# aagbotemi/zk-cryptography

Measured on AMD Instinct MI355X. Metric: field-evals/s (sumcheck 2^24) + MSM points/s (KZG 2^20) per BASELINE.json; value = the sumcheck prover's field-evals/s, the MSM half is under "msm", higher is better.
Workload: dtype u32; 1 GPU; 24-var multilinear sumcheck prover (poly_sum + prove), BLS12-381 Fr; field=BLS12-381 Fr (255-bit Montgomery, 8 x u32 limbs); G1 over Fq (381-bit), evals_per_gpu=16777216, exchanges_per_prove=0

## Files before the change

zk-cryptography_amd/csrc/ctx.hpp:

```cpp
#pragma once
#include <hip/hip_runtime.h>
#include <stdint.h>

#include <algorithm>
#include <deque>
#include <functional>
#include <memory>
#include <mutex>
#include <new>
#include <set>
#include <vector>

#include "../../include/zkhip.h"
#include "hip_own.hpp"
#include "host_util.hpp"

#define ZK_MAX_ROUNDS 48
#define ZK_MAX_PARTIALS 4096

enum : size_t {
    ZK_SMALL_R = 0,
    ZK_SMALL_RES = 16,
    ZK_SMALL_STATE = 64,
    ZK_SMALL_PTS = 256,
    ZK_SMALL_CHALLENGES = ZK_SMALL_PTS + 4 * ZK_MAX_ROUNDS,
    ZK_SMALL_ROUNDPOLYS = ZK_SMALL_CHALLENGES + 4 * ZK_MAX_ROUNDS,
    ZK_SMALL_PARTIALS = ZK_SMALL_ROUNDPOLYS + 64 * ZK_MAX_ROUNDS,
    ZK_SMALL_END = ZK_SMALL_PARTIALS + 4 * 8 * ZK_MAX_PARTIALS
};
#define ZK_SMALL_BYTES (ZK_SMALL_END * 8)

enum : size_t {
    ZK_PIN_R = 0,
    ZK_PIN_RES = 16,
    ZK_PIN_PTS = 64,
    ZK_PIN_PROOF = ZK_PIN_PTS + 4 * ZK_MAX_ROUNDS,
    ZK_PIN_END = ZK_PIN_PROOF + 4 + 8 * ZK_MAX_ROUNDS + 4 * ZK_MAX_ROUNDS + 64 * ZK_MAX_ROUNDS
};
#define ZK_PINNED_BYTES (ZK_PIN_END * 8)

#define ZK_HIP(ctx, call)                                   \
    do {                                                    \
        hipError_t _e = (call);                             \
        if (_e != hipSuccess) {                             \
            (ctx)->last_hip = (int)_e;                      \
            return ZKHIP_ERR_HIP;                           \
        }                                                   \
    } while (0)
#define ZK_TRY(expr)                 \
    do {                             \
        int _s = (expr);             \
        if (_s != ZKHIP_OK) return _s; \
    } while (0)

struct ZkProfEvent { zk::Event start, stop; };
struct ZkProfRecord { const char* name; size_t event; double bytes; };

struct NttCache;
struct NttCacheDelete { void operator()(NttCache*) const; };
struct MsmPending;
struct MsmPendingDelete { void operator()(MsmPending*) const; };
namespace zk { struct MsmGeometry; }
struct ZkCtxDestroy { void operator()(zkhip_ctx* c) const { (void)zkhip_ctx_destroy(c); } };
using ZkCtxOwner = std::unique_ptr<zkhip_ctx, ZkCtxDestroy>;

struct zkhip_ctx {
    int device = 0;
    hipStream_t stream = nullptr;
    zk::Stream owned_stream;
    int last_hip = 0;
    zk::GrowBuf ws;
    zk::DevMem d_fingerprint;
    zk::Stream guard_stream;
    zk::Event guard_ev;
    zk::DevMem d_composed;
    zk::DevMem d_gen_table;
    std::unique_ptr<NttCache, NttCacheDelete> ntt_state;
    zk::GrowBuf aux;
    uint32_t outer_token = 0;
    static constexpr int MSM_SLOTS = 6;
    zk::GrowBuf msm_pin[MSM_SLOTS];
    zk::Event msm_ev[MSM_SLOTS];
    zk::Stream side[MSM_SLOTS];
    zk::Event fork_ev, join_ev, serial_ev;
    int ensure_side_streams() {
        for (int i = 0; i < MSM_SLOTS; ++i)
            if (zk::ensure_stream(side[i]) != hipSuccess) return ZKHIP_ERR_HIP;
// ... 82 lines not shown
    }
    int ensure_lane(int k, size_t ws_need) {
        ProofLane& L = lanes[k];
        { const int rc = ensure_lane_streams(k); if (rc != ZKHIP_OK) return rc; }
        { const int rc = ensure_lane_fold(k); if (rc != ZKHIP_OK) return rc; }
        if (zk::ensure_event(L.begin_ev) != hipSuccess || zk::ensure_event(L.fork_ev) != hipSuccess || zk::ensure_event(L.serial_ev) != hipSuccess) return ZKHIP_ERR_HIP;
        if (!L.small && zk::dev_alloc(L.small, ZK_SMALL_BYTES) != hipSuccess) return ZKHIP_ERR_NOMEM;
        if (L.ws.ptr) return L.ws.reserve(ws_need, {L.serial, L.fold});
        return L.ws.reserve(ws_need);
    }
    int reserve_msm_pin(int slot, size_t bytes) {
        if (zk::ensure_event(msm_ev[slot]) != hipSuccess) return ZKHIP_ERR_HIP;
        return msm_pin[slot].reserve_pinned(bytes);
    }
    zk::GrowBuf msm_tab_dev[MSM_SLOTS], msm_tab_pin[MSM_SLOTS];
    std::shared_ptr<const zk::MsmGeometry> msm_tab_geo[MSM_SLOTS];
    int reserve_msm_tab(int slot, size_t bytes) {
        const size_t cap = (bytes + 65535) & ~(size_t)65535;
        if (cap > msm_tab_dev[slot].bytes || cap > msm_tab_pin[slot].bytes) msm_tab_geo[slot].reset();
        ZK_TRY(msm_tab_dev[slot].reserve(cap));
        return msm_tab_pin[slot].reserve_pinned(cap);
    }
    std::vector<ZkCtxOwner> gkr_lanes;
    bool gkr_lane = false;
    zkhip_ctx* gkr_parent = nullptr;
    std::mutex gkr_warm_mu;
    zk::GrowBuf gkr_in;
    struct GkrGraph {
        zk::GraphExec exec;
        const void *cir = nullptr, *aux = nullptr, *in = nullptr, *ws = nullptr, *pin = nullptr, *composed = nullptr;
        const void *warm_cir = nullptr, *warm_aux = nullptr, *warm_ws = nullptr;
    } gkr_graph;
    ZkLoanDesk ws_loans;
    static constexpr int ASYNC_SLOTS = 3;
    std::unique_ptr<MsmPending, MsmPendingDelete> async_pend[ASYNC_SLOTS];
    size_t async_region = 0;
    zk::DevMem sc_small, sc_stage; size_t sc_stage_cap = 0;
    ZkLoanDesk sc_loans;
    zk::DevMem d_small;
    zk::PinMem h_pinned;
    bool profiling = false;
    std::vector<ZkProfEvent> prof_events;
    size_t prof_used = 0;
    std::vector<ZkProfRecord> prof_records;

    int activate() {
        hipError_t e = hipSetDevice(device);
        if (e != hipSuccess) { last_hip = (int)e; return ZKHIP_ERR_HIP; }
        return ZKHIP_OK;
    }
    std::set<const void*> big_lds_done;
    int allow_big_lds(const void* fn, size_t bytes) {
        if (bytes <= 64 * 1024 || big_lds_done.count(fn)) return ZKHIP_OK;
        hipError_t e = hipFuncSetAttribute(fn, hipFuncAttributeMaxDynamicSharedMemorySize, (int)bytes);
        if (e != hipSuccess) { last_hip = (int)e; return ZKHIP_ERR_HIP; }
        big_lds_done.insert(fn);
        return ZKHIP_OK;
    }
    zk::Event done_ev;
    int wait_stream(hipStream_t s = nullptr) {
        if (!s) s = stream;
        if (zk::ensure_event(done_ev) != hipSuccess) return ZKHIP_ERR_HIP;
        if (hipEventRecord(done_ev.get(), s) != hipSuccess) return ZKHIP_ERR_HIP;
        if (s != stream && hipStreamWaitEvent(stream, done_ev.get(), 0) != hipSuccess) return ZKHIP_ERR_HIP;
        for (int spin = 0; spin < 200000; ++spin) {
            const hipError_t e = hipEventQuery(done_ev.get());
            if (e == hipSuccess) return ZKHIP_OK;
            if (e != hipErrorNotReady) { last_hip = (int)e; return ZKHIP_ERR_HIP; }
        }
        const hipError_t e = hipStreamSynchronize(s);
        if (e != hipSuccess) { last_hip = (int)e; return ZKHIP_ERR_HIP; }
        return ZKHIP_OK;
    }
    int wait_event(hipEvent_t ev) {
        for (int spin = 0; spin < 200000; ++spin) {
            const hipError_t e = hipEventQuery(ev);
            if (e == hipSuccess) return ZKHIP_OK;
            if (e != hipErrorNotReady) { last_hip = (int)e; return ZKHIP_ERR_HIP; }
        }
        const hipError_t e = hipEventSynchronize(ev);
        if (e != hipSuccess) { last_hip = (int)e; return ZKHIP_ERR_HIP; }
        return ZKHIP_OK;
    }
    zk::PinMem proof_pin[PROOF_SLOTS];
    zk::Event proof_ev[PROOF_SLOTS];
    uint32_t proof_pending[PROOF_SLOTS] = {};
    int ensure_proof_slot(int k) {
        if (zk::ensure_event(proof_ev[k]) != hipSuccess) return ZKHIP_ERR_HIP;
        if (!proof_pin[k] && zk::pin_alloc(proof_pin[k], ((ZK_SMALL_ROUNDPOLYS - ZK_SMALL_STATE) + 8 * ZK_MAX_ROUNDS) * 8) != hipSuccess) return ZKHIP_ERR_NOMEM;
        return ZKHIP_OK;
    }
    void drain_streams() {
        hipStreamSynchronize(stream);
        if (fold_stream) hipStreamSynchronize(fold_stream.get());
        for (auto& L : lanes) { if (L.serial) hipStreamSynchronize(L.serial); if (L.fold) hipStreamSynchronize(L.fold); }
        for (auto& s : side) if (s) hipStreamSynchronize(s.get());
        if (guard_stream) hipStreamSynchronize(guard_stream.get());
    }
    uint64_t* small_u64(size_t off) { return (uint64_t*)d_small.get() + off; }
    uint64_t* pinned_u64(size_t off) { return (uint64_t*)h_pinned.get() + off; }
    int reserve_aux(size_t bytes) { return aux.reserve(bytes, {stream}, &last_hip); }
    int reserve_ws(size_t bytes) {
        if (ws_loans.lent()) return ZKHIP_ERR_BUSY;
        return ws.reserve(bytes, {stream}, &last_hip);
    }
    std::unique_ptr<ZkHostPool> host_pool;
    ZkHostPool* pool() {
        if (!host_pool) {
            const unsigned hw = std::max(1u, std::thread::hardware_concurrency());
            host_pool.reset(new (std::nothrow) ZkHostPool(std::min(hw, 32u) - 1));
        }
        return host_pool.get();
    }
};

struct ProfScope {
    zkhip_ctx* c;
    size_t idx = 0;
    bool on;
    hipStream_t s;
    ProfScope(zkhip_ctx* ctx, const char* name, double bytes, hipStream_t on_stream = nullptr)
        : c(ctx), on(ctx->profiling), s(on_stream ? on_stream : ctx->stream) {
        if (!on) return;
        if (c->prof_used == c->prof_events.size()) {
            ZkProfEvent ev;
            (void)zk::ensure_event(ev.start, hipEventDefault);
            (void)zk::ensure_event(ev.stop, hipEventDefault);
            c->prof_events.push_back(std::move(ev));
        }
        idx = c->prof_used++;
        hipEventRecord(c->prof_events[idx].start.get(), s);
        c->prof_records.push_back({name, idx, bytes});
    }
    ~ProfScope() {
        if (on) hipEventRecord(c->prof_events[idx].stop.get(), s);
    }
};

int zk_ntt_scaled_transform(zkhip_ctx* c, const uint64_t* d_src, size_t n_src, const uint64_t* d_mul, uint64_t* d_dst, uint32_t log_n);
bool zk_msm_commit_batch_serves(size_t n_points, size_t longest);
int zk_msm_commit_batch(zkhip_ctx* c, const void* d_table_with_header, const uint8_t* d_points_inf, size_t n_points, const uint64_t* d_scalars,
                        size_t q_stride, uint32_t batch, uint32_t m, const size_t* sc_off, const size_t* lens, uint64_t* h_out_xy,
                        uint8_t* h_out_inf, size_t out_stride);
```

zk-cryptography_amd/csrc/diag_all.hip:

```cpp
#include "zkhip.hip"
#include "composed.hip"
#include "gkr.hip"
#include "ntt.hip"
#include "shard.hip"
extern "C" int zkhip_kzg_commit(zkhip_ctx*, const uint64_t*, const uint8_t*, size_t, const uint64_t*, size_t, int, uint64_t*, uint8_t*) { return ZKHIP_ERR_ARG; }
extern "C" int zkhip_kzg_commit_table(zkhip_ctx*, const void*, const uint8_t*, size_t, const uint64_t*, size_t, int, uint64_t*, uint8_t*) { return ZKHIP_ERR_ARG; }
extern "C" int zkhip_kzg_commit_end(zkhip_ctx*, uint32_t, uint64_t*, uint8_t*) { return ZKHIP_ERR_ARG; }
extern "C" int zkhip_g1_sum_affine(const uint64_t*, const uint8_t*, size_t, uint64_t*, uint8_t*) { return ZKHIP_ERR_ARG; }
void MsmPendingDelete::operator()(MsmPending*) const {}
```

zk-cryptography_amd/csrc/multifold_kernels.hpp:

```cpp
#pragma once
#include "sumcheck_kernels.hpp"
#include "wide_acc.hpp"

namespace zk {

constexpr int MF_MAX_LOGK = 8;
constexpr int MF_CAP_LOGK = 9;

static __global__ __launch_bounds__(MLE_BLOCK) void chunk_sums_kernel(const uint64_t* __restrict__ in, uint32_t chunk,
                                                                      uint64_t* __restrict__ partials) {
    __shared__ Fr red[MLE_BLOCK / 64];
    const uint64_t* base = in + 4 * (size_t)blockIdx.x * chunk;
    Fr s = Fr::zero();
    for (uint32_t j = threadIdx.x; j < chunk; j += 4 * MLE_BLOCK) {
        Fr v[4];
#pragma unroll
        for (int u = 0; u < 4; ++u) v[u] = (j + u * MLE_BLOCK < chunk) ? load_fr(base, j + u * MLE_BLOCK) : Fr::zero();
#pragma unroll
        for (int u = 0; u < 4; ++u) s = s + v[u];
    }
    s = block_reduce_fr(s, red);
    if (threadIdx.x == 0) store_fr(partials, blockIdx.x, s);
}

static __global__ __launch_bounds__(MLE_BLOCK) void group_sums_kernel(const uint64_t* __restrict__ partials, uint32_t group,
                                                                      uint32_t n_blocks, uint64_t* __restrict__ out) {
    __shared__ Fr red[MLE_BLOCK / 64];
    Fr tot = Fr::zero();
    for (uint32_t b = threadIdx.x; b < n_blocks; b += MLE_BLOCK) {
        Fr s = Fr::zero();
        for (uint32_t g = 0; g < group; ++g) s = s + load_fr(partials, (size_t)b * group + g);
        store_fr(out, b, s);
        tot = tot + s;
    }
    tot = block_reduce_fr(tot, red);
    if (threadIdx.x == 0) store_fr(out, n_blocks, tot);
}

constexpr int FINE_CHUNK = 256;
static __global__ __launch_bounds__(MLE_BLOCK) void fine_sums_kernel(const uint64_t* __restrict__ in, size_t n_chunks,
                                                                     uint64_t* __restrict__ sums) {
    const uint32_t lane = threadIdx.x & 63, wave = threadIdx.x >> 6;
    const size_t c0 = ((size_t)blockIdx.x * (MLE_BLOCK / 64) + wave) * 2;
    if (c0 >= n_chunks) return;
    const bool two = c0 + 1 < n_chunks;
    const uint64_t* base = in + 4 * (c0 * FINE_CHUNK);
    Fr v[8];
#pragma unroll
    for (int u = 0; u < 4; ++u) v[u] = load_fr(base, lane + 64 * u);
#pragma unroll
    for (int u = 4; u < 8; ++u) v[u] = two ? load_fr(base, lane + 64 * u) : Fr::zero();
    Fr a = (v[0] + v[1]) + (v[2] + v[3]);
    Fr b = (v[4] + v[5]) + (v[6] + v[7]);
    wave_reduce_fr2(a, b);
    if (lane == 0) {
        store_fr(sums, c0, a);
        if (two) store_fr(sums, c0 + 1, b);
    }
}

static __global__ __launch_bounds__(MLE_BLOCK) void group_sums_wg_kernel(const uint64_t* __restrict__ in, uint32_t group,
                                                                         uint64_t* __restrict__ out_mont, uint64_t* __restrict__ out_canon) {
    __shared__ Fr red[MLE_BLOCK / 64];
    const uint64_t* base = in + 4 * (size_t)blockIdx.x * group;
    Fr s = Fr::zero();
    for (uint32_t j = threadIdx.x; j < group; j += 4 * MLE_BLOCK) {
        Fr v[4];
#pragma unroll
        for (int u = 0; u < 4; ++u) v[u] = (j + u * MLE_BLOCK < group) ? load_fr(base, j + u * MLE_BLOCK) : Fr::zero();
#pragma unroll
        for (int u = 0; u < 4; ++u) s = s + v[u];
    }
    s = block_reduce_fr(s, red);
    if (threadIdx.x == 0) {
        if (out_mont) store_fr(out_mont, blockIdx.x, s);
        if (out_canon) store_fr(out_canon, blockIdx.x, fr_from_mont_outlined(s));
    }
}

constexpr int TREE_MAX_LOG = 10;

struct SmallArgs {
    const uint64_t* src;
    uint32_t group;
    uint32_t stride;
    uint32_t canon;
    uint32_t log_n;
    uint32_t n_rounds;
    uint32_t round0;
    uint32_t first;
    FrArg claimed;
    const uint64_t* d_claimed;
    uint64_t* weights_out;
    uint64_t* final_out;
    long long host_delta;
};

constexpr int SMALL_BLOCK = 512;

static __global__ __launch_bounds__(SMALL_BLOCK) void sumcheck_small_kernel(SmallArgs a, SumcheckDev* st,
                                                                            uint64_t* __restrict__ round_polys,
                                                                            uint64_t* __restrict__ challenges) {
    extern __shared__ __attribute__((aligned(16))) unsigned char zk_dyn_lds[];
    __builtin_amdgcn_s_setprio(3);
    ZK_STAMP_AT(0, 40 + a.round0, 0);
    const uint32_t n = 1u << a.log_n;
    Fr* tree0 = reinterpret_cast<Fr*>(zk_dyn_lds);
    Fr* tree1 = tree0 + 2 * n;
    const uint32_t w_all = a.weights_out ? (1u << a.n_rounds) : 0u;
    Fr* w0 = tree1 + n;
    Fr* w1 = w0 + ((a.n_rounds & 1) ? w_all / 2 : w_all);
    const bool grouped = a.group != 0 && a.stride == 0;
    Fr* scratch = w0 + w_all + w_all / 2 + 1;
    Fr* e_sh = scratch + (grouped ? SMALL_BLOCK : 0);
    Fr* r_sh = e_sh + 4;
    if (a.host_delta && a.round0) {
        for (uint32_t i = threadIdx.x; i < 12 * a.round0 + 4; i += SMALL_BLOCK) {
            const uint64_t* p = i < 4 ? st->sum + i : i < 4 + 8 * a.round0 ? round_polys + (i - 4) : challenges + (i - 4 - 8 * a.round0);
            *const_cast<uint64_t*>(p + a.host_delta) = *p;
        }
    }
    if (a.group == 0) {
        for (uint32_t j = threadIdx.x; j < n; j += SMALL_BLOCK) {
            const Fr v = load_fr(a.src, j);
            tree0[n + j] = a.canon ? v : fr_from_mont_outlined(v);
        }
    } else if (a.stride != 0) {
        for (uint32_t j = threadIdx.x; j < n; j += SMALL_BLOCK) {
            Fr s = load_fr(a.src, j);
            for (uint32_t g = 1; g < a.group; g += 8) {
                Fr v[8];
#pragma unroll
                for (int u = 0; u < 8; ++u) if (g + u < a.group) v[u] = load_fr(a.src, (size_t)(g + u) * a.stride + j);
#pragma unroll
                for (int u = 0; u < 8; ++u) if (g + u < a.group) s = s + v[u];
            }
            tree0[n + j] = a.canon ? s : fr_from_mont_outlined(s);
        }
    } else {
        const uint32_t total = n * a.group;
        const uint32_t run = total > (uint32_t)SMALL_BLOCK ? total / SMALL_BLOCK : 1;
        if (threadIdx.x * run < total) {
            Fr s = Fr::zero();
            for (uint32_t g = 0; g < run; ++g) s = s + load_fr(a.src, (size_t)threadIdx.x * run + g);
            scratch[threadIdx.x] = s;
        }
        __syncthreads();
        const uint32_t tpe = a.group / run;
        for (uint32_t j = threadIdx.x; j < n; j += SMALL_BLOCK) {
            Fr s = scratch[j * tpe];
            for (uint32_t g = 1; g < tpe; ++g) s = s + scratch[j * tpe + g];
            tree0[n + j] = a.canon ? s : fr_from_mont_outlined(s);
        }
    }
    if (threadIdx.x == 0 && a.weights_out) {
        Fr one32;
        constexpr uint32_t c[8] = {0xcaaf6b13u, 0x355094eau, 0x69a568efu, 0xf6b10cb3u, 0x40cc3869u, 0xe2c926a6u, 0xed269aadu, 0x736a6d3bu};
#pragma unroll
        for (int i = 0; i < 8; ++i) one32.l[i] = c[i];
        w0[0] = one32;
    }
    __syncthreads();
    for (uint32_t lvl = a.log_n; lvl > 1;) {
        const uint32_t step = lvl - 1 < 3 ? lvl - 1 : 3;
        const uint32_t groups = 1u << (lvl - step);
        for (uint32_t g = threadIdx.x; g < groups; g += SMALL_BLOCK) {
            Fr v[8];
            const uint32_t cnt0 = 1u << step;
#pragma unroll
            for (int i = 0; i < 8; ++i) if ((uint32_t)i < cnt0) v[i] = tree0[(1u << lvl) + g * cnt0 + i];
#pragma unroll
            for (int sft = 1; sft <= 3; ++sft) {
                if ((uint32_t)sft <= step) {
                    const uint32_t cnt = cnt0 >> sft;
#pragma unroll
                    for (int i = 0; i < 4; ++i) {
                        if ((uint32_t)i < cnt) {
                            v[i] = v[2 * i] + v[2 * i + 1];
                            tree0[(1u << (lvl - sft)) + g * cnt + i] = v[i];
                        }
                    }
                }
            }
        }
        __syncthreads();
        lvl -= step;
    }
    const uint32_t wave = threadIdx.x >> 6;
    const bool wave0 = wave == 0;
    uint32_t* kw1 = reinterpret_cast<uint32_t*>(r_sh + 2);
    uint32_t* kw2 = kw1 + 64;
    uint32_t* dig_sh = kw2 + 64;
    uint32_t* flags = dig_sh + 16;
    if (threadIdx.x >= 64 && threadIdx.x < 66 && a.log_n >= 2)
        e_sh[threadIdx.x - 64] = (tree0[6 + threadIdx.x - 64] - tree0[4 + threadIdx.x - 64]).to_mont();
    if (threadIdx.x == 0) {
        flags[0] = 0; flags[1] = 0;
        uint32_t pre[8];
        if (a.first) {
            const Fr sum_c = (a.first == 2) ? fr_from_mont_outlined(fr_from_arg(a.claimed))
                           : (a.first == 3) ? fr_from_mont_outlined(load_fr(a.d_claimed, 0)) : tree0[2] + tree0[3];
#pragma unroll
            for (int i = 0; i < 8; ++i) pre[i] = sum_c.l[7 - i];
        } else {
#pragma unroll
            for (int i = 0; i < 8; ++i) pre[i] = st->transcript.buf[i];
        }
#pragma unroll
        for (int i = 0; i < 8; ++i) dig_sh[8 + i] = pre[i];
    }
    __syncthreads();
    Fr lo = tree0[2], hi = tree0[3];
    uint32_t depth = a.log_n, round = a.round0, n_w = 1;
    ZK_STAMP_AT(0, 40 + a.round0, 1);
    const uint32_t word = threadIdx.x & 15;
    auto schedule_block1 = [&](const uint32_t* prefix, const Fr& lo_c, uint32_t it) {
        const uint32_t w = word < 8 ? prefix[word] : fr_limb_by_lane(lo_c, 15 - word);
        sha256_schedule_rows_to_lds(w, kw1, flags, 4 * it, 1, threadIdx.x < 64 + 16);
    };
    auto schedule_block2 = [&](const Fr& hi_c, uint32_t it) {
        const uint32_t w = word < 8 ? fr_limb_by_lane(hi_c, 7 - word) : (word == 8 ? 0x80000000u : word == 15 ? 96u * 8u : 0u);
        sha256_schedule_rows_to_lds(w, kw2, flags + 1, 4 * it, 0, threadIdx.x < 128 + 16);
    };
    if (a.n_rounds) {
        if (wave == 1) schedule_block1(dig_sh + 8, lo, 0);
        if (wave == 2) schedule_block2(hi, 0);
    }
    uint32_t digest[8];
    constexpr uint32_t FIRST_HELPER = 192, N_HELPERS = SMALL_BLOCK - FIRST_HELPER - 64, OUT_WAVE = 4;
    if (wave == OUT_WAVE) __builtin_amdgcn_s_setprio(0);
    for (uint32_t it = 0; it < a.n_rounds; ++it) {
        Fr* told = (it & 1) ? tree1 : tree0;
        Fr* tnew = (it & 1) ? tree0 : tree1;
        Fr* wold = (it & 1) ? w1 : w0;
        Fr* wnew = (it & 1) ? w0 : w1;
        Fr* eold = e_sh + 2 * (it & 1);
        Fr* enew = e_sh + 2 * ((it & 1) ^ 1);
        const bool absorb_sum = a.first && it == 0;
        if (wave0) {
            ZK_STAMP_AT(0, round, 0);
            uint32_t h[8] = {0x6a09e667u, 0xbb67ae85u, 0x3c6ef372u, 0xa54ff53au, 0x510e527fu, 0x9b05688cu, 0x1f83d9abu, 0x5be0cd19u};
            uint32_t blk[16];
            const uint32_t* pre = dig_sh + 8 * ((it + 1) & 1);
#pragma unroll
            for (int i = 0; i < 8; ++i) { blk[i] = pre[i]; blk[8 + i] = lo.l[7 - i]; }
            ShaSplit sp;
            sp.init();
            uint32_t hs[4];
            sp.split(h, hs);
            sha256_compress_kw_split(sp, hs, blk, kw1, flags, 4 * it);
            ZK_STAMP_AT(0, round, 1);
            sha256_compress_kw_split(sp, hs, nullptr, kw2, flags + 1, 4 * it);
            sp.join(hs, h);
            ZK_STAMP_AT(0, round, 2);
#pragma unroll
            for (int i = 0; i < 8; ++i) digest[i] = h[i];
            Fr c;
#pragma unroll
            for (int i = 0; i < 8; ++i) c.l[i] = h[7 - i];
            c.reduce_once();
            c.reduce_once();
            if (threadIdx.x == 0) {
                r_sh[it & 1] = c;
#pragma unroll
                for (int i = 0; i < 8; ++i) dig_sh[8 * (it & 1) + i] = h[i];
            }
        }
        ZK_STAMP_AT(0, round, 3);
        ZK_STAMP_AT(SMALL_BLOCK - 1, round, 6);
        ZK_STAMP_AT(64, round, 7);
        __syncthreads();
        ZK_STAMP_AT(0, round, 4);
        const Fr c = r_sh[it & 1];
        if (wave0) {
            if (depth >= 2) {
                const uint32_t q = threadIdx.x & 1;
                Fr v = told[4 + q] + fr_mul_outlined(c, eold[q]);
                lo = shfl_fr(v, 0);
                hi = shfl_fr(v, 1);
            }
            ZK_STAMP_AT(0, round, 5);
        } else if (wave <= 2) {
            if (it + 1 < a.n_rounds && depth >= 2) {
                const uint32_t q = wave - 1;
                const Fr v = told[4 + q] + fr_mul_outlined(c, eold[q]);
                if (wave == 1) schedule_block1(dig_sh + 8 * (it & 1), v, it + 1);
                else schedule_block2(v, it + 1);
            }
        } else {
            const Fr r = fr_to_mont_outlined(c);
            const uint32_t helper = wave == OUT_WAVE ? N_HELPERS : wave < OUT_WAVE ? threadIdx.x - FIRST_HELPER : threadIdx.x - FIRST_HELPER - 64;
            if (threadIdx.x == 64 * OUT_WAVE) {
                Fr lo_m = told[2].to_mont(), hi_m = told[3].to_mont();
                if (absorb_sum) {
                    Fr sum_m = (a.first == 2) ? fr_from_arg(a.claimed) : (a.first == 3) ? load_fr(a.d_claimed, 0) : lo_m + hi_m;
                    store_fr(st->sum, 0, sum_m);
                    if (a.host_delta) store_fr(st->sum + a.host_delta, 0, sum_m);
                }
                store_fr(round_polys, 2 * (size_t)round, lo_m);
                store_fr(round_polys, 2 * (size_t)round + 1, hi_m);
                store_fr(challenges, round, r);
                if (a.host_delta) {
                    store_fr(round_polys + a.host_delta, 2 * (size_t)round, lo_m);
                    store_fr(round_polys + a.host_delta, 2 * (size_t)round + 1, hi_m);
                    store_fr(challenges + a.host_delta, round, r);
                }
            }
            const uint32_t nodes = 1u << (depth - 1);
            if (helper >= N_HELPERS - 2 && helper < N_HELPERS && depth >= 3) {
                const uint32_t q = 4 + (helper - (N_HELPERS - 2));
                Fr va = told[q + 4] + r * (told[q + 8] - told[q + 4]);
                Fr vb = told[q + 6] + r * (told[q + 10] - told[q + 6]);
                tnew[q] = va;
                tnew[q + 2] = vb;
                enew[helper - (N_HELPERS - 2)] = (vb - va).to_mont();
            }
            for (uint32_t q = 1 + helper; q < 2 * nodes && helper < N_HELPERS; q += N_HELPERS) {
                if (depth >= 3 && q >= 4 && q < 8) continue;
                const uint32_t p = 1u << (31 - __builtin_clz(q));
                tnew[q] = told[q + p] + r * (told[q + 2 * p] - told[q + p]);
            }
            if (a.weights_out) {
                for (uint32_t b = helper; b < n_w && helper < N_HELPERS; b += N_HELPERS) {
                    Fr w1v = wold[b] * r;
                    wnew[2 * b + 1] = w1v;
                    wnew[2 * b] = wold[b] - w1v;
                }
            }
        }
        n_w <<= 1;
        --depth;
        ++round;
    }
    ZK_STAMP_AT(0, 40 + a.round0, 2);
    __syncthreads();
    if (threadIdx.x == 0 && a.n_rounds) {
        Transcript tr;
        tr.init();
        tr.commit_words8(digest);
        tr.store(&st->transcript);
    }

    if (a.weights_out) {
        Fr* w = (a.n_rounds & 1) ? w1 : w0;
        for (uint32_t b = threadIdx.x; b < n_w; b += SMALL_BLOCK) store_fr(a.weights_out, b, w[b]);
    }
    if (a.final_out) {
        Fr* t = (a.n_rounds & 1) ? tree1 : tree0;
        const uint32_t cnt = 1u << depth;
        for (uint32_t j = threadIdx.x; j < cnt; j += SMALL_BLOCK) store_fr(a.final_out, j, t[cnt + j].to_mont());
    }
}
__host__ __device__ constexpr size_t small_lds_bytes(uint32_t log_n, int weight_rounds, bool grouped) {
    return ((size_t)3 * ((size_t)1 << log_n) + (weight_rounds >= 0 ? 3 * ((size_t)1 << weight_rounds) / 2 : 0u) + 1 +
            (grouped ? SMALL_BLOCK : 0) + 4 + 2) * 32 + (64 + 64 + 16 + 2) * 4;
}

static __global__ __launch_bounds__(MLE_BLOCK) void eq_weights_kernel(PtsArg pts, uint32_t first, uint32_t k,
                                                                      uint64_t* __restrict__ out) {
    const uint32_t b = blockIdx.x * MLE_BLOCK + threadIdx.x;
    if (b >= (1u << k)) return;
    Fr w;
    constexpr uint32_t c[8] = {0xcaaf6b13u, 0x355094eau, 0x69a568efu, 0xf6b10cb3u, 0x40cc3869u, 0xe2c926a6u, 0xed269aadu, 0x736a6d3bu};
#pragma unroll
    for (int i = 0; i < 8; ++i) w.l[i] = c[i];
    const Fr one = Fr::one();
    for (uint32_t i = 0; i < k; ++i) {
        Fr r = fr_from_pts(pts, first + i);
        if (!((b >> (k - 1 - i)) & 1)) r = one - r;
        w = w * r;
    }
    store_fr(out, b, w);
}

static __global__ __launch_bounds__(MLE_BLOCK) void eval_weights_kernel(PtsArg pts, uint32_t k1, uint32_t k2, uint32_t s, uint64_t* __restrict__ w1,
                                                                        uint64_t* __restrict__ wa, uint64_t* __restrict__ wb) {
    size_t b = (size_t)blockIdx.x * MLE_BLOCK + threadIdx.x;
    const size_t n1 = (size_t)1 << k1, na = (size_t)1 << (k2 - s), nb = (size_t)1 << s;
    uint32_t k, first;
    uint64_t* out;
    Fr w = Fr::one();
    if (b < n1) {
        k = k1; first = 0; out = w1;
        constexpr uint32_t c[8] = {0xcaaf6b13u, 0x355094eau, 0x69a568efu, 0xf6b10cb3u, 0x40cc3869u, 0xe2c926a6u, 0xed269aadu, 0x736a6d3bu};
#pragma unroll
        for (int i = 0; i < 8; ++i) w.l[i] = c[i];
    } else if (b < n1 + na) {
        b -= n1; k = k2 - s; first = k1; out = wa;
    } else if (b < n1 + na + nb) {
        b -= n1 + na; k = s; first = k1 + k2 - s; out = wb;
    } else {
        return;
    }
    const Fr one = Fr::one();
    for (uint32_t i = 0; i < k; ++i) {
        Fr r = fr_from_pts(pts, first + i);
        if (!((b >> (k - 1 - i)) & 1)) r = one - r;
        w = w * r;
    }
    store_fr(out, b, w);
}
static __global__ __launch_bounds__(MLE_BLOCK) void sum_records_kernel(const uint64_t* __restrict__ records, uint32_t n, uint64_t* __restrict__ out) {
    __shared__ Fr red[MLE_BLOCK / 64];
    Fr s = Fr::zero();
    for (uint32_t i = threadIdx.x; i < n; i += 4 * MLE_BLOCK) {
        Fr v[4];
#pragma unroll
        for (int u = 0; u < 4; ++u) v[u] = (i + u * MLE_BLOCK < n) ? load_fr(records, i + u * MLE_BLOCK) : Fr::zero();
#pragma unroll
        for (int u = 0; u < 4; ++u) s = s + v[u];
    }
    s = block_reduce_fr(s, red);
    if (threadIdx.x == 0) store_fr(out, 0, s);
}

template <int G, int DEPTH = 4, bool NT = false>
static __global__ __launch_bounds__(1024) void multifold_kernel(const uint64_t* __restrict__ in, size_t m, uint32_t k,
                                                                const uint64_t* __restrict__ weights,
// ... 116 lines not shown
```

zk-cryptography_amd/csrc/zkhip.hip:

```cpp
#include "../../include/zkhip.h"

#include <hip/hip_runtime.h>

#include <algorithm>
#include <cstdio>
#include <cstdlib>
#include <cstring>
#include <map>
#include <string>
#include <vector>

#include "ctx.hpp"
#include "host_util.hpp"
#include "mle_kernels.hpp"
#include "sumcheck_kernels.hpp"
#include "multifold_kernels.hpp"
#include "mfma_fold.hpp"
#include "tunables.hpp"

using namespace zk;

static int g_last_hip = 0;
extern "C" int zkhip_version(void) { return 1; }

// ... 553 lines not shown
        uint64_t* d_chunk = nullptr;
        if (m > (size_t)FINE_CHUNK) { ZK_TRY(c->reserve_ws((n / FINE_CHUNK) * 32)); d_chunk = (uint64_t*)c->ws.ptr; }
        ZK_TRY(launch_fine_sums(c, d_evals, n, log_blocks, d_out, d_chunk));
        if (want_total) {
            const uint32_t k1 = overlapped_plan(n) && log_blocks == log2_exact(n) - 8 ? log_blocks - overlapped_k2(n) : 8;
            int cs = 0;
            ZK_TRY(c->next_coarse(&cs));
            uint64_t* coarse_canon = (uint64_t*)c->d_coarse[cs].get(), *coarse_mont = coarse_canon + 4 * 1024;
            {
                ProfScope ps(c, "coarse_sums", 0.0);
                hipLaunchKernelGGL(group_sums_wg_kernel, dim3(1u << k1), dim3(MLE_BLOCK), 0, c->stream, d_out, 1u << (log_blocks - k1), coarse_mont, coarse_canon);
            }
            {
                ProfScope ps(c, "total_sum", 0.0);
                hipLaunchKernelGGL(group_sums_wg_kernel, dim3(1), dim3(MLE_BLOCK), 0, c->stream, coarse_mont, 1u << k1, d_out + 4 * ((size_t)1 << log_blocks), (uint64_t*)nullptr);
            }
            c->coarse_of[cs] = d_out; c->coarse_n[cs] = n; c->coarse_k1[cs] = k1;
        }
    } else {
        const size_t n_chunks = n / std::min<size_t>(m, 4096);
        uint64_t* d_partials;
        if (n_chunks <= 8 * (size_t)ZK_MAX_PARTIALS) d_partials = c->small_u64(ZK_SMALL_PARTIALS);
        else { ZK_TRY(c->reserve_ws(n_chunks * 32)); d_partials = (uint64_t*)c->ws.ptr; }
        const uint64_t* parts = nullptr;
        const uint32_t group = launch_chunk_sums(c, c->stream, d_evals, n, m, d_partials, &parts);
        hipLaunchKernelGGL(group_sums_kernel, dim3(1), dim3(MLE_BLOCK), 0, c->stream, parts, group, 1u << log_blocks, d_out);
    }
    ZK_HIP(c, hipGetLastError());
    if (h_total) {
        ZK_HIP(c, hipMemcpyAsync(c->pinned_u64(ZK_PIN_RES), d_out + 4 * ((size_t)1 << log_blocks), 32, hipMemcpyDeviceToHost, c->stream));
        ZK_HIP(c, hipStreamSynchronize(c->stream));
        std::memcpy(h_total, c->pinned_u64(ZK_PIN_RES), 32);
    }
    return ZKHIP_OK;
}

extern "C" int zkhip_mle_block_sums(zkhip_ctx* c, const uint64_t* d_evals, size_t n, uint32_t log_blocks,
                                    uint64_t* d_out, uint64_t* h_total) {
    return block_sums_impl(c, d_evals, n, log_blocks, d_out, h_total, true);
}
extern "C" int zkhip_mle_block_sums_deferred(zkhip_ctx* c, const uint64_t* d_evals, size_t n, uint32_t log_blocks, uint64_t* d_out) {
    return block_sums_impl(c, d_evals, n, log_blocks, d_out, nullptr, false);
}
extern "C" int zkhip_mle_block_sums_total(zkhip_ctx* c, uint64_t* d_block_sums, uint32_t log_blocks, uint64_t* h_total) {
    if (!c || !d_block_sums || !h_total || log_blocks > 16) return ZKHIP_ERR_ARG;
    ZK_TRY(c->activate());
    const uint32_t hi = log_blocks / 2, lo = log_blocks - hi;
    uint64_t* tmp = c->small_u64(ZK_SMALL_PARTIALS);
    hipLaunchKernelGGL(group_sums_wg_kernel, dim3(1u << hi), dim3(MLE_BLOCK), 0, c->stream, d_block_sums, 1u << lo, tmp, (uint64_t*)nullptr);
    hipLaunchKernelGGL(group_sums_wg_kernel, dim3(1), dim3(MLE_BLOCK), 0, c->stream, tmp, 1u << hi, d_block_sums + 4 * ((size_t)1 << log_blocks), (uint64_t*)nullptr);
    ZK_HIP(c, hipGetLastError());
    ZK_HIP(c, hipMemcpyAsync(c->pinned_u64(ZK_PIN_RES), d_block_sums + 4 * ((size_t)1 << log_blocks), 32, hipMemcpyDeviceToHost, c->stream));
    ZK_HIP(c, hipStreamSynchronize(c->stream));
    std::memcpy(h_total, c->pinned_u64(ZK_PIN_RES), 32);
    return ZKHIP_OK;
}

struct ProofLayout { size_t tabA, tabB, partA, partB, w, w2, fine, p1, p2, total; };
constexpr ProofLayout proof_layout(size_t n, bool overlap) {
    const size_t part = n / 256 + 1024, w = (size_t)1 << TREE_MAX_LOG;
    ProofLayout l = {};
    l.tabA = 0;
    l.tabB = (overlap ? n / 8 : n / 4) + 32;
    l.partA = (overlap ? n / 8 : n / 4 + n / 16) + 64;
    l.partB = l.partA + part;
    l.w = l.partB + part;
    l.w2 = l.w + w;
    l.fine = l.w2 + w;
    l.p1 = l.fine + SC_FINE_ENTRIES;
    l.p2 = l.p1 + SC_P1_ENTRIES;
    l.total = overlap ? l.p2 + SC_P2_ENTRIES : l.fine;
    return l;
}
static_assert(proof_layout((size_t)1 << 24, true).tabB == 2097184 && proof_layout((size_t)1 << 24, true).partA == 2097216 &&
              proof_layout((size_t)1 << 24, true).total == 2230336 + (2 << TREE_MAX_LOG) + 65536 + 2048 + 8192,
              "the bench size's tables have moved");
struct ProofRun {
    hipStream_t S, F;
    hipEvent_t fork_ev, serial_ev;
    uint64_t *tabA, *tabB, *partA, *partB, *w, *w2, *fine, *p1, *p2;
    SumcheckDev* st;
    uint64_t *d_rp, *d_ch, *d_fin;
    long long host_delta;
    uint32_t round;
    const uint64_t *h_claimed, *d_claimed;
    SmallArgs rounds(const uint64_t* src, uint32_t group, uint32_t stride, uint32_t canon, uint32_t k, uint64_t* weights_out) {
        SmallArgs a = small_rounds(src, group, stride, canon, k, k, round, weights_out);
        small_open(a, round == 0, h_claimed, d_claimed);
        round += k;
        return a;
    }
    SmallArgs closing_rounds(const uint64_t* src, uint32_t group, uint32_t stride, uint32_t canon, uint32_t k) {
        SmallArgs a = rounds(src, group, stride, canon, k, nullptr);
        a.final_out = d_fin; a.host_delta = host_delta;
        return a;
    }
};
static int proof_setup(zkhip_ctx* c, size_t n, bool overlap, const uint64_t* h_claimed_sum, const uint64_t* d_claimed_sum, int slot, int lane,
                       ProofRun& p) {
    const ProofLayout l = proof_layout(n, overlap);
    const size_t ws_need = l.total * 32;
    p = {};
    uint64_t *ws, *small;
    if (lane < 0) {
        ZK_TRY(c->reserve_ws(ws_need));
        ws = (uint64_t*)c->ws.ptr; small = (uint64_t*)c->d_small.get(); p.S = c->stream;
        if (overlap) { ZK_TRY(c->ensure_fold_stream()); p.F = c->fold_stream.get(); p.fork_ev = c->fork_ev.get(); p.serial_ev = c->serial_ev.get(); }
    } else {
        ZK_TRY(c->ensure_lane(lane, ws_need));
        zkhip_ctx::ProofLane& L = c->lanes[lane];
        ws = (uint64_t*)L.ws.ptr; small = (uint64_t*)L.small.get(); p.S = L.serial; p.F = L.fold; p.fork_ev = L.fork_ev.get(); p.serial_ev = L.serial_ev.get();
        ZK_HIP(c, hipEventRecord(L.begin_ev.get(), c->stream));
        ZK_HIP(c, hipStreamWaitEvent(p.S, L.begin_ev.get(), 0));
    }
    p.tabA = ws + 4 * l.tabA; p.tabB = ws + 4 * l.tabB; p.partA = ws + 4 * l.partA; p.partB = ws + 4 * l.partB;
    p.w = ws + 4 * l.w; p.w2 = ws + 4 * l.w2; p.fine = ws + 4 * l.fine; p.p1 = ws + 4 * l.p1; p.p2 = ws + 4 * l.p2;
    p.st = (SumcheckDev*)(small + ZK_SMALL_STATE);
    p.d_rp = small + ZK_SMALL_ROUNDPOLYS;
    p.d_ch = small + ZK_SMALL_CHALLENGES;
    p.d_fin = small + ZK_SMALL_RES;
    ZK_TRY(c->ensure_proof_slot(slot));
    p.host_delta = ((long long)(intptr_t)c->proof_pin[slot].get() - (long long)(intptr_t)(small + ZK_SMALL_STATE)) / 8;
    p.h_claimed = h_claimed_sum; p.d_claimed = d_claimed_sum;
    return ZKHIP_OK;
}
static int proof_last_stage(zkhip_ctx* c, ProofRun p, hipStream_t stream, uint32_t k2) {
    uint32_t ny = 0;
    ZK_TRY(launch_blockfold(c, stream, p.tabA, 256, k2, p.w2, p.p2, &ny));
    return launch_small(c, p.closing_rounds(p.p2, ny, 256, 1, 8), p.st, p.d_rp, p.d_ch, 0, stream);
}
static int proof_overlapped(zkhip_ctx* c, ProofRun& p, const uint64_t* d_evals, size_t n, const uint64_t* d_block_sums, uint32_t log_blocks,
                            int slot, int lane, int in_flight, hipStream_t* tail) {
    const uint32_t g = log2_exact(n) - 8, k2 = overlapped_k2(n), k1 = g - k2;
    const hipStream_t S = p.S;
    const uint64_t* fine = d_block_sums;
    if (!fine || log_blocks != g) {
        const bool on_callers = lane >= 0 && in_flight >= 3;
        ZK_TRY(launch_fine_sums(c, d_evals, n, g, p.fine, nullptr, on_callers ? c->stream : S));
        if (on_callers) {
            ZK_HIP(c, hipEventRecord(c->lanes[lane].begin_ev.get(), c->stream));
            ZK_HIP(c, hipStreamWaitEvent(S, c->lanes[lane].begin_ev.get(), 0));
        }
        fine = p.fine;
    }
    int cs = -1;
    for (int q = 1; q <= zkhip_ctx::COARSE_RING && cs < 0; ++q) {
        const int e = (c->coarse_next - q + 2 * zkhip_ctx::COARSE_RING) % zkhip_ctx::COARSE_RING;
        if (fine == d_block_sums && c->coarse_of[e] == fine && c->coarse_n[e] == n && c->coarse_k1[e] == k1) cs = e;
    }
    if (cs < 0) {
        ZK_TRY(c->next_coarse(&cs));
        ProfScope ps(c, "coarse_sums", 0.0, S);
        hipLaunchKernelGGL(group_sums_wg_kernel, dim3(1u << k1), dim3(MLE_BLOCK), 0, S, fine, 1u << k2, (uint64_t*)nullptr, (uint64_t*)c->d_coarse[cs].get());
    }
    const uint64_t* coarse = (const uint64_t*)c->d_coarse[cs].get();
    c->coarse_of[cs] = nullptr;
    c->coarse_owner[cs] = slot + 1;
    ZK_TRY(launch_small(c, p.rounds(coarse, 0, 0, 1, k1, p.w), p.st, p.d_rp, p.d_ch, 0, S));
    uint32_t ny = 0, n_parts = 0;
    ZK_TRY(launch_blockfold(c, S, fine, 1u << k2, k1, p.w, p.p1, &ny));
    ZK_HIP(c, hipEventRecord(p.fork_ev, S));
    const SmallArgs b = p.rounds(p.p1, ny, 1u << k2, 1, k2, p.w2);
    if (lane >= 0 && in_flight < 3) { ZK_TRY(c->ensure_lane_fold(lane)); p.F = c->lanes[lane].fold; }
    if (lane >= 0 && in_flight >= 3) {
        ZK_TRY(launch_small(c, b, p.st, p.d_rp, p.d_ch, 156 * 1024, S));
        c->deferred_rc[slot] = ZKHIP_OK;
        const ProofRun held = p;
        c->deferred.emplace_back(slot, [c, held, d_evals, n, k1, k2, slot]() -> int {
            uint32_t np2 = 0;
            ZK_HIP(c, hipStreamWaitEvent(c->stream, held.fork_ev, 0));
            ZK_TRY(launch_multifold(c, c->stream, d_evals, n, k1, held.w, held.tabA, held.partA, &np2));
            ZK_HIP(c, hipEventRecord(held.serial_ev, c->stream));
            ZK_HIP(c, hipStreamWaitEvent(held.S, held.serial_ev, 0));
            ZK_TRY(proof_last_stage(c, held, held.S, k2));
            ZK_HIP(c, hipEventRecord(c->proof_ev[slot].get(), held.S));
            return ZKHIP_OK;
        });
        (void)c->flush_deferred((size_t)std::min(3, std::max(1, in_flight - 3)));
        *tail = nullptr;
        return ZKHIP_OK;
    }
    ZK_HIP(c, hipStreamWaitEvent(p.F, p.fork_ev, 0));
    ZK_TRY(launch_multifold(c, p.F, d_evals, n, k1, p.w, p.tabA, p.partA, &n_parts));
    ZK_TRY(launch_small(c, b, p.st, p.d_rp, p.d_ch, 156 * 1024, S));
    ZK_HIP(c, hipEventRecord(p.serial_ev, S));
    ZK_HIP(c, hipStreamWaitEvent(p.F, p.serial_ev, 0));
    *tail = p.F;
    return proof_last_stage(c, p, p.F, k2);
}
static int proof_stages(zkhip_ctx* c, ProofRun& p, const uint64_t* d_evals, size_t n, const uint64_t* d_block_sums, uint32_t log_blocks) {
    const uint64_t* cur = d_evals;
    size_t cn = n;
    const uint64_t* parts = nullptr;
    uint32_t n_parts = 0;
    for (uint32_t stage = 0; stage_k(cn) != 0; ++stage) {
        const uint32_t k = stage_k(cn);
        const size_t m = cn >> k;
        uint32_t group;
        if (stage == 0 && d_block_sums && log_blocks >= k && log_blocks <= (uint32_t)MF_CAP_LOGK) {
            parts = d_block_sums;
            group = 1u << (log_blocks - k);
        } else if (stage == 0) {
            group = launch_chunk_sums(c, p.S, cur, cn, m, p.partA, &parts);
        } else {
            group = (uint32_t)(n_parts >> k);
        }
        ZK_TRY(launch_small(c, p.rounds(parts, group, 0, 0, k, p.w), p.st, p.d_rp, p.d_ch, 0, p.S));
        uint64_t* dst = (stage & 1) ? p.tabB : p.tabA;
        uint64_t* pdst = (stage & 1) ? p.partB : p.partA;
        ZK_TRY(launch_multifold(c, p.S, cur, cn, k, p.w, dst, pdst, &n_parts));
        parts = pdst;
        cur = dst;
        cn = m;
    }
    return launch_small(c, p.closing_rounds(cur, 0, 0, 0, log2_exact(cn)), p.st, p.d_rp, p.d_ch, 0, p.S);
}
static int sumcheck_enqueue(zkhip_ctx* c, const uint64_t* d_evals, size_t n, const uint64_t* h_claimed_sum,
                            const uint64_t* d_claimed_sum, const uint64_t* d_block_sums, uint32_t log_blocks, int slot, int lane, int in_flight = 1) {
    const bool overlap = overlapped_plan(n);
    ProofRun p;
    ZK_TRY(proof_setup(c, n, overlap, h_claimed_sum, d_claimed_sum, slot, lane, p));
    hipStream_t tail_stream = p.S;
    if (overlap) {
        ZK_TRY(proof_overlapped(c, p, d_evals, n, d_block_sums, log_blocks, slot, lane, in_flight, &tail_stream));
        if (!tail_stream) return ZKHIP_OK;
    } else {
        ZK_TRY(proof_stages(c, p, d_evals, n, d_block_sums, log_blocks));
    }
    ZK_HIP(c, hipEventRecord(c->proof_ev[slot].get(), tail_stream));
    if (lane < 0 && tail_stream != c->stream) ZK_HIP(c, hipStreamWaitEvent(c->stream, c->proof_ev[slot].get(), 0));
    return ZKHIP_OK;
}
static int sumcheck_collect(zkhip_ctx* c, int slot, uint32_t n_vars, uint64_t* h_sum, uint64_t* h_round_polys, uint64_t* h_challenges) {
    const int wrc = c->wait_event(c->proof_ev[slot].get());
    c->release_coarse(slot);
    ZK_TRY(wrc);
    const uint64_t* pin = (const uint64_t*)c->proof_pin[slot].get();
    const uint64_t* span = c->small_u64(ZK_SMALL_STATE);
    const SumcheckDev* st = (const SumcheckDev*)c->small_u64(ZK_SMALL_STATE);
    std::memcpy(h_sum, pin + ((const uint64_t*)st->sum - span), 32);
    std::memcpy(h_round_polys, pin + (c->small_u64(ZK_SMALL_ROUNDPOLYS) - span), 64 * (size_t)n_vars);
    std::memcpy(h_challenges, pin + (c->small_u64(ZK_SMALL_CHALLENGES) - span), 32 * (size_t)n_vars);
    return ZKHIP_OK;
}
static int sumcheck_check_args(zkhip_ctx* c, const uint64_t* d_evals, size_t n) {
    if (!c || !d_evals) return ZKHIP_ERR_ARG;
    if (!is_pow2(n)) return ZKHIP_ERR_SHAPE;
    if (log2_exact(n) > ZK_MAX_ROUNDS) return ZKHIP_ERR_SHAPE;
    return ZKHIP_OK;
}

extern "C" int zkhip_sumcheck_prove(zkhip_ctx* c, const uint64_t* d_evals, size_t n, const uint64_t* h_claimed_sum,
                                    const uint64_t* d_claimed_sum, const uint64_t* d_block_sums, uint32_t log_blocks,
                                    uint64_t* h_sum,
                                    uint64_t* h_round_polys, uint64_t* h_challenges) {
    ZK_TRY(sumcheck_check_args(c, d_evals, n));
    if (!h_sum) return ZKHIP_ERR_ARG;
    const uint32_t n_vars = log2_exact(n);
    if (n_vars && (!h_round_polys || !h_challenges)) return ZKHIP_ERR_ARG;
    for (int k = 0; k < zkhip_ctx::PROOF_SLOTS; ++k) if (c->proof_pending[k]) return ZKHIP_ERR_BUSY;
    ZK_TRY(c->activate());
    if (n == 1) {
        if (h_claimed_sum) { std::memcpy(h_sum, h_claimed_sum, 32); return ZKHIP_OK; }
        ZK_HIP(c, hipMemcpyAsync(c->pinned_u64(ZK_PIN_RES), d_claimed_sum ? d_claimed_sum : d_evals, 32, hipMemcpyDeviceToHost, c->stream));
        ZK_HIP(c, hipStreamSynchronize(c->stream));
        std::memcpy(h_sum, c->pinned_u64(ZK_PIN_RES), 32);
        return ZKHIP_OK;
    }
    ZK_TRY(sumcheck_enqueue(c, d_evals, n, h_claimed_sum, d_claimed_sum, d_block_sums, log_blocks, 0, -1));
    return sumcheck_collect(c, 0, n_vars, h_sum, h_round_polys, h_challenges);
}
extern "C" int zkhip_sumcheck_prove_begin(zkhip_ctx* c, const uint64_t* d_evals, size_t n, const uint64_t* h_claimed_sum,
                                          const uint64_t* d_claimed_sum, const uint64_t* d_block_sums, uint32_t log_blocks,
                                          uint32_t* ticket) {
    ZK_TRY(sumcheck_check_args(c, d_evals, n));
    if (!ticket || n < 2) return ZKHIP_ERR_ARG;
    int slot = -1;
    for (int k = 0; k < zkhip_ctx::PROOF_SLOTS; ++k) if (!c->proof_pending[k]) { slot = k; break; }
    if (slot < 0) return ZKHIP_ERR_BUSY;
    ZK_TRY(c->activate());
    int in_flight = 1;
    for (int k = 0; k < zkhip_ctx::PROOF_SLOTS; ++k) in_flight += c->proof_pending[k] != 0;
    ZK_TRY(sumcheck_enqueue(c, d_evals, n, h_claimed_sum, d_claimed_sum, d_block_sums, log_blocks, slot, slot, in_flight));
    c->proof_pending[slot] = log2_exact(n);
    *ticket = (uint32_t)slot;
    return ZKHIP_OK;
}
extern "C" int zkhip_sumcheck_prove_end(zkhip_ctx* c, uint32_t ticket, uint64_t* h_sum, uint64_t* h_round_polys, uint64_t* h_challenges) {
    if (!c || ticket >= (uint32_t)zkhip_ctx::PROOF_SLOTS || !c->proof_pending[ticket]) return ZKHIP_ERR_ARG;
    const uint32_t n_vars = c->proof_pending[ticket];
    int rc = c->activate();
    if (rc == ZKHIP_OK) {
        (void)c->flush_deferred(0, (int)ticket);
        rc = c->deferred_rc[ticket];
        c->deferred_rc[ticket] = ZKHIP_OK;
        if (rc != ZKHIP_OK) {
            (void)hipStreamSynchronize(c->lanes[ticket].serial);
            (void)hipStreamSynchronize(c->stream);
            c->release_coarse((int)ticket);
        }
    }
    if (rc == ZKHIP_OK) {
        if (h_sum && h_round_polys && h_challenges) rc = sumcheck_collect(c, (int)ticket, n_vars, h_sum, h_round_polys, h_challenges);
        else { rc = c->wait_event(c->proof_ev[ticket].get()); c->release_coarse((int)ticket); }
        if (hipStreamWaitEvent(c->stream, c->proof_ev[ticket].get(), 0) != hipSuccess && rc == ZKHIP_OK) rc = ZKHIP_ERR_HIP;
    }
    c->proof_pending[ticket] = 0;
    return rc;
}

struct zkhip_sc_state {
    zkhip_ctx* c;
    const uint64_t* cur;
    size_t cn;
    uint64_t *A, *B;
    uint64_t* small;
    uint32_t round, np;
    bool partials_valid;
    DevMem own_tables, own_small, own_stage;
    ZkLoan ws_loan, sc_loan;
    uint64_t* stage_buf;
    size_t stage_parts_cap;
    uint32_t stage_k_cur, stage_world, stage_idx, n_parts;
    const uint64_t* parts;
    uint32_t ov_k1 = 0, ov_k2 = 0, ov_ny1 = 0, ov_phase = 0;
    uint64_t* ov_fine() { return B; }
    uint64_t* ov_w1() { return B + 4 * SC_FINE_ENTRIES; }
    uint64_t* ov_w2() { return ov_w1() + 4 * ((size_t)1 << TREE_MAX_LOG); }
    uint64_t* ov_p2() { return ov_w2() + 4 * ((size_t)1 << TREE_MAX_LOG); }
    uint64_t* ov_loc() { return ov_p2() + 4 * SC_P2_ENTRIES; }
    uint64_t* sw() { return stage_buf; }
    uint64_t* spx() { return stage_buf + 4 * ((size_t)1 << MF_CAP_LOGK); }
    uint64_t* spy() { return spx() + 4 * stage_parts_cap; }
    uint64_t* sbs() { return spy() + 4 * stage_parts_cap; }
    SumcheckDev* dev() { return (SumcheckDev*)small; }
    uint64_t* rp() { return small + 64; }
    uint64_t* ch() { return rp() + 8 * ZK_MAX_ROUNDS; }
    uint64_t* partials() { return ch() + 4 * ZK_MAX_ROUNDS; }
    uint64_t* fin() { return partials() + 8 * (size_t)MLE_MAX_GRID; }
};

extern "C" int zkhip_sc_begin(zkhip_ctx* c, const uint64_t* d_local, size_t n_local, zkhip_sc_state** out) {
    if (!c || !d_local || !out) return ZKHIP_ERR_ARG;
    if (!is_pow2(n_local)) return ZKHIP_ERR_SHAPE;
    ZK_TRY(c->activate());
    std::unique_ptr<zkhip_sc_state> st(new zkhip_sc_state());
    st->c = c; st->cur = d_local; st->cn = n_local; st->round = 0; st->np = 0; st->partials_valid = false;
    st->A = st->B = st->small = st->stage_buf = nullptr;
    const size_t small_u64 = 64 + 12 * (size_t)ZK_MAX_ROUNDS + 8 * (size_t)MLE_MAX_GRID + 16;
    st->stage_parts_cap = std::max<size_t>(n_local / 256, 64) + 64;
    if (!c->sc_loans.lent() && c->sc_small && c->sc_stage_cap >= st->stage_parts_cap) {
        st->sc_loan = ZkLoan(c->sc_loans);
        st->stage_parts_cap = c->sc_stage_cap;
    } else {
        if (dev_alloc(st->own_small, small_u64 * 8) != hipSuccess) return ZKHIP_ERR_NOMEM;
        if (dev_alloc(st->own_stage, (((size_t)1 << MF_CAP_LOGK) + 2 * st->stage_parts_cap + ((size_t)1 << MF_CAP_LOGK) + 1 + 8) * 32) != hipSuccess) return ZKHIP_ERR_NOMEM;
    }
    st->small = (uint64_t*)(st->sc_loan ? c->sc_small : st->own_small).get();
    st->stage_buf = (uint64_t*)(st->sc_loan ? c->sc_stage : st->own_stage).get();
    if (n_local >= 2) {
        const size_t bytes = (n_local / 2 + n_local / 4 + 4) * 32;
        if (!c->ws_loans.lent()) {
            ZK_TRY(c->reserve_ws(bytes));
            st->A = (uint64_t*)c->ws.ptr;
            st->ws_loan = ZkLoan(c->ws_loans);
        } else {
            if (dev_alloc(st->own_tables, bytes) != hipSuccess) return ZKHIP_ERR_NOMEM;
            st->A = (uint64_t*)st->own_tables.get();
        }
    }
    st->B = st->A ? st->A + 4 * (n_local / 2) : nullptr;
    st->stage_k_cur = 0; st->stage_world = 1; st->stage_idx = 0; st->n_parts = 0; st->parts = nullptr;
    *out = st.release();
    return ZKHIP_OK;
}

int zk_sc_plan_stage(size_t cn, uint32_t world, uint32_t* k_out) {
    if (!k_out || !is_pow2(world) || !is_pow2(cn)) return ZKHIP_ERR_ARG;
    uint32_t k;
    if (world == 1) {
        k = stage_k(cn);
    } else {
        const uint32_t lg = log2_exact(cn * world);
        const uint32_t tail_log = log2_exact((size_t)zkhip_sc_tail_capacity());
        if (lg <= tail_log) k = 0;
        else {
// ... 322 lines not shown
```

Measured before the change: 54.51 billion field-evals/s.

## Signal sumcheck completion via pinned sequence word polled by host

The closing small kernel now writes a per-slot sequence number to pinned host memory with a system-scope release store. The synchronous prove path spins on that word with a short timeout before falling back to the event, so it skips event-completion latency. The host copy-out of earlier round data moves from the kernel prologue to the low-priority output wave, and the grouped strided load loop is restructured into branch-free unrolled loads. The risk is that the host reads pinned results before the event completes, which depends on release/acquire ordering being correct. It also calls release_coarse before the stream may be fully drained.

```diff
diff --git a/zk-cryptography_amd/csrc/ctx.hpp b/zk-cryptography_amd/csrc/ctx.hpp
--- a/zk-cryptography_amd/csrc/ctx.hpp
+++ b/zk-cryptography_amd/csrc/ctx.hpp
@@ -3,6 +3,7 @@
 #include <stdint.h>
 
 #include <algorithm>
+#include <chrono>
 #include <deque>
 #include <functional>
 #include <memory>
@@ -251,13 +252,31 @@
         if (e != hipSuccess) { last_hip = (int)e; return ZKHIP_ERR_HIP; }
         return ZKHIP_OK;
     }
+    static constexpr size_t PROOF_PIN_WORDS = (ZK_SMALL_ROUNDPOLYS - ZK_SMALL_STATE) + 8 * ZK_MAX_ROUNDS;
     zk::PinMem proof_pin[PROOF_SLOTS];
     zk::Event proof_ev[PROOF_SLOTS];
     uint32_t proof_pending[PROOF_SLOTS] = {};
+    uint64_t proof_seq[PROOF_SLOTS] = {};
+    uint64_t* proof_word(int k) { return (uint64_t*)proof_pin[k].get() + PROOF_PIN_WORDS; }
     int ensure_proof_slot(int k) {
         if (zk::ensure_event(proof_ev[k]) != hipSuccess) return ZKHIP_ERR_HIP;
-        if (!proof_pin[k] && zk::pin_alloc(proof_pin[k], ((ZK_SMALL_ROUNDPOLYS - ZK_SMALL_STATE) + 8 * ZK_MAX_ROUNDS) * 8) != hipSuccess) return ZKHIP_ERR_NOMEM;
-        return ZKHIP_OK;
+        if (!proof_pin[k]) {
+            if (zk::pin_alloc(proof_pin[k], (PROOF_PIN_WORDS + 8) * 8) != hipSuccess) return ZKHIP_ERR_NOMEM;
+            *proof_word(k) = 0;
+        }
+        return ZKHIP_OK;
+    }
+    int wait_proof(int k) {
+        if (!profiling) {
+            const volatile uint64_t* word = proof_word(k);
+            const uint64_t want = proof_seq[k];
+            const auto give_up = std::chrono::steady_clock::now() + std::chrono::milliseconds(2);
+            do {
+                for (int spin = 0; spin < 256; ++spin)
+                    if (__atomic_load_n(word, __ATOMIC_ACQUIRE) == want) return ZKHIP_OK;
+            } while (std::chrono::steady_clock::now() < give_up);
+        }
+        return wait_event(proof_ev[k].get());
     }
     void drain_streams() {
         hipStreamSynchronize(stream);
diff --git a/zk-cryptography_amd/csrc/diag_all.hip b/zk-cryptography_amd/csrc/diag_all.hip
--- a/zk-cryptography_amd/csrc/diag_all.hip
+++ b/zk-cryptography_amd/csrc/diag_all.hip
@@ -6,5 +6,6 @@
 extern "C" int zkhip_kzg_commit(zkhip_ctx*, const uint64_t*, const uint8_t*, size_t, const uint64_t*, size_t, int, uint64_t*, uint8_t*) { return ZKHIP_ERR_ARG; }
 extern "C" int zkhip_kzg_commit_table(zkhip_ctx*, const void*, const uint8_t*, size_t, const uint64_t*, size_t, int, uint64_t*, uint8_t*) { return ZKHIP_ERR_ARG; }
 extern "C" int zkhip_kzg_commit_end(zkhip_ctx*, uint32_t, uint64_t*, uint8_t*) { return ZKHIP_ERR_ARG; }
+extern "C" int zkhip_table_release(zkhip_ctx*, const void*) { return ZKHIP_OK; }
 extern "C" int zkhip_g1_sum_affine(const uint64_t*, const uint8_t*, size_t, uint64_t*, uint8_t*) { return ZKHIP_ERR_ARG; }
 void MsmPendingDelete::operator()(MsmPending*) const {}
diff --git a/zk-cryptography_amd/csrc/multifold_kernels.hpp b/zk-cryptography_amd/csrc/multifold_kernels.hpp
--- a/zk-cryptography_amd/csrc/multifold_kernels.hpp
+++ b/zk-cryptography_amd/csrc/multifold_kernels.hpp
@@ -94,6 +94,8 @@
     uint64_t* weights_out;
     uint64_t* final_out;
     long long host_delta;
+    uint64_t seq;
+    uint64_t* seq_word;
 };
 
 constexpr int SMALL_BLOCK = 512;
@@ -114,12 +116,6 @@
     Fr* scratch = w0 + w_all + w_all / 2 + 1;
     Fr* e_sh = scratch + (grouped ? SMALL_BLOCK : 0);
     Fr* r_sh = e_sh + 4;
-    if (a.host_delta && a.round0) {
-        for (uint32_t i = threadIdx.x; i < 12 * a.round0 + 4; i += SMALL_BLOCK) {
-            const uint64_t* p = i < 4 ? st->sum + i : i < 4 + 8 * a.round0 ? round_polys + (i - 4) : challenges + (i - 4 - 8 * a.round0);
-            *const_cast<uint64_t*>(p + a.host_delta) = *p;
-        }
-    }
     if (a.group == 0) {
         for (uint32_t j = threadIdx.x; j < n; j += SMALL_BLOCK) {
             const Fr v = load_fr(a.src, j);
@@ -127,13 +123,17 @@
         }
     } else if (a.stride != 0) {
         for (uint32_t j = threadIdx.x; j < n; j += SMALL_BLOCK) {
-            Fr s = load_fr(a.src, j);
-            for (uint32_t g = 1; g < a.group; g += 8) {
+            Fr s;
+            for (uint32_t g = 0; g < a.group; g += 8) {
                 Fr v[8];
 #pragma unroll
-                for (int u = 0; u < 8; ++u) if (g + u < a.group) v[u] = load_fr(a.src, (size_t)(g + u) * a.stride + j);
-#pragma unroll
-                for (int u = 0; u < 8; ++u) if (g + u < a.group) s = s + v[u];
+                for (int u = 0; u < 8; ++u) {
+                    const uint32_t gu = g + u < a.group ? g + u : a.group - 1;
+                    v[u] = load_fr(a.src, (size_t)gu * a.stride + j);
+                }
+                if (g == 0) s = v[0];
+#pragma unroll
+                for (int u = 0; u < 8; ++u) if (g + u < a.group && g + u != 0) s = s + v[u];
             }
             tree0[n + j] = a.canon ? s : fr_from_mont_outlined(s);
         }
@@ -228,7 +228,15 @@
     }
     uint32_t digest[8];
     constexpr uint32_t FIRST_HELPER = 192, N_HELPERS = SMALL_BLOCK - FIRST_HELPER - 64, OUT_WAVE = 4;
-    if (wave == OUT_WAVE) __builtin_amdgcn_s_setprio(0);
+    if (wave == OUT_WAVE) {
+        __builtin_amdgcn_s_setprio(0);
+        if (a.host_delta && a.round0) {
+            for (uint32_t i = threadIdx.x - 64 * OUT_WAVE; i < 12 * a.round0 + 4; i += 64) {
+                const uint64_t* p = i < 4 ? st->sum + i : i < 4 + 8 * a.round0 ? round_polys + (i - 4) : challenges + (i - 4 - 8 * a.round0);
+                *const_cast<uint64_t*>(p + a.host_delta) = *p;
+            }
+        }
+    }
     for (uint32_t it = 0; it < a.n_rounds; ++it) {
         Fr* told = (it & 1) ? tree1 : tree0;
         Fr* tnew = (it & 1) ? tree0 : tree1;
@@ -333,7 +341,12 @@
         ++round;
     }
     ZK_STAMP_AT(0, 40 + a.round0, 2);
+    if (a.seq_word && wave == OUT_WAVE) __builtin_amdgcn_fence(__ATOMIC_RELEASE, "");
     __syncthreads();
+    if (a.seq_word && threadIdx.x == 64 * OUT_WAVE) {
+        __hip_atomic_store(a.seq_word, a.seq, __ATOMIC_RELEASE, __HIP_MEMORY_SCOPE_SYSTEM);
+        ZK_STAMP_AT(64 * OUT_WAVE, 40 + a.round0, 3);
+    }
     if (threadIdx.x == 0 && a.n_rounds) {
         Transcript tr;
         tr.init();
diff --git a/zk-cryptography_amd/csrc/zkhip.hip b/zk-cryptography_amd/csrc/zkhip.hip
--- a/zk-cryptography_amd/csrc/zkhip.hip
+++ b/zk-cryptography_amd/csrc/zkhip.hip
@@ -659,6 +659,8 @@
     SumcheckDev* st;
     uint64_t *d_rp, *d_ch, *d_fin;
     long long host_delta;
+    uint64_t seq;
+    uint64_t* seq_word;
     uint32_t round;
     const uint64_t *h_claimed, *d_claimed;
     SmallArgs rounds(const uint64_t* src, uint32_t group, uint32_t stride, uint32_t canon, uint32_t k, uint64_t* weights_out) {
@@ -669,7 +671,7 @@
     }
     SmallArgs closing_rounds(const uint64_t* src, uint32_t group, uint32_t stride, uint32_t canon, uint32_t k) {
         SmallArgs a = rounds(src, group, stride, canon, k, nullptr);
-        a.final_out = d_fin; a.host_delta = host_delta;
+        a.final_out = d_fin; a.host_delta = host_delta; a.seq = seq; a.seq_word = seq_word;
         return a;
     }
 };
@@ -698,6 +700,8 @@
     p.d_fin = small + ZK_SMALL_RES;
     ZK_TRY(c->ensure_proof_slot(slot));
     p.host_delta = ((long long)(intptr_t)c->proof_pin[slot].get() - (long long)(intptr_t)(small + ZK_SMALL_STATE)) / 8;
+    p.seq = ++c->proof_seq[slot];
+    p.seq_word = c->proof_word(slot);
     p.h_claimed = h_claimed_sum; p.d_claimed = d_claimed_sum;
     return ZKHIP_OK;
 }
@@ -808,8 +812,8 @@
     if (lane < 0 && tail_stream != c->stream) ZK_HIP(c, hipStreamWaitEvent(c->stream, c->proof_ev[slot].get(), 0));
     return ZKHIP_OK;
 }
-static int sumcheck_collect(zkhip_ctx* c, int slot, uint32_t n_vars, uint64_t* h_sum, uint64_t* h_round_polys, uint64_t* h_challenges) {
-    const int wrc = c->wait_event(c->proof_ev[slot].get());
+static int sumcheck_collect(zkhip_ctx* c, int slot, uint32_t n_vars, uint64_t* h_sum, uint64_t* h_round_polys, uint64_t* h_challenges, bool by_word) {
+    const int wrc = by_word ? c->wait_proof(slot) : c->wait_event(c->proof_ev[slot].get());
     c->release_coarse(slot);
     ZK_TRY(wrc);
     const uint64_t* pin = (const uint64_t*)c->proof_pin[slot].get();
@@ -845,7 +849,7 @@
         return ZKHIP_OK;
     }
     ZK_TRY(sumcheck_enqueue(c, d_evals, n, h_claimed_sum, d_claimed_sum, d_block_sums, log_blocks, 0, -1));
-    return sumcheck_collect(c, 0, n_vars, h_sum, h_round_polys, h_challenges);
+    return sumcheck_collect(c, 0, n_vars, h_sum, h_round_polys, h_challenges, true);
 }
 extern "C" int zkhip_sumcheck_prove_begin(zkhip_ctx* c, const uint64_t* d_evals, size_t n, const uint64_t* h_claimed_sum,
                                           const uint64_t* d_claimed_sum, const uint64_t* d_block_sums, uint32_t log_blocks,
@@ -878,7 +882,7 @@
         }
     }
     if (rc == ZKHIP_OK) {
-        if (h_sum && h_round_polys && h_challenges) rc = sumcheck_collect(c, (int)ticket, n_vars, h_sum, h_round_polys, h_challenges);
+        if (h_sum && h_round_polys && h_challenges) rc = sumcheck_collect(c, (int)ticket, n_vars, h_sum, h_round_polys, h_challenges, false);
         else { rc = c->wait_event(c->proof_ev[ticket].get()); c->release_coarse((int)ticket); }
         if (hipStreamWaitEvent(c->stream, c->proof_ev[ticket].get(), 0) != hipSuccess && rc == ZKHIP_OK) rc = ZKHIP_ERR_HIP;
     }
```

After: 57.32 billion field-evals/s, median of 6. 1.05x the previous value.
